# kfirc1503/generative-audio

Hardware: AMD Instinct MI355X
Metric: spectrogram-frames/sec, NPPC K=5 FullSubNet+ train step (higher is better)
Workload: dtype bf16

## Files before the change

generative-audio_amd/csrc/spec.hip:

```cpp
#include "common.h"
#include "nppc_hip.h"

namespace {

struct MapSet { const float* x[6]; };

template <bool RAGGED>
__global__ __launch_bounds__(256) void rowsum_kernel(MapSet ms, double* __restrict__ sums, const int* __restrict__ frames, long R,
                                                     int C, int T) {
  const long r = (long)blockIdx.x * 4 + (threadIdx.x >> 6);
  if (r >= R) return;
  const int lane = threadIdx.x & 63;
  const int Tb = RAGGED ? clampi(frames[r / C], 1, T) : T;
  const float* x = ms.x[blockIdx.y];
  sums += (size_t)blockIdx.y * R;
  const float* p = x + (size_t)r * T;
  double s = 0.0;
  for (int t = lane; t < Tb; t += 64) s += (double)p[t];
  s = wave_sum(s);
  if (lane == 0) sums[r] = s;
}

struct TsseW {
  const float* cw[3];
  const float* cb[3];
  int ks[3];
  const float* fcw;
  const float* fcb;
  const float* w1;
  const float* b1;
  const float* w2;
  const float* b2;
};

constexpr int TSSE_MAXC = 1024;
__device__ __forceinline__ TsseW tsse_branch(TsseW w, long off) {
  for (int i = 0; i < 3; ++i) { w.cw[i] += off; if (w.cb[i]) w.cb[i] += off; }
  w.fcw += off; if (w.fcb) w.fcb += off;
  w.w1 += off; if (w.b1) w.b1 += off;
  w.w2 += off; if (w.b2) w.b2 += off;
  return w;
}

template <bool RAGGED>
__global__ __launch_bounds__(1024) void tsse_fwd_kernel(MapSet ms, const double* __restrict__ rowsum,
                                                       TsseW w, long sW, int nm, float* __restrict__ scale, float* __restrict__ ns_out,
                                                       float* __restrict__ pre_out, float* __restrict__ sq_out,
                                                       float* __restrict__ h1_out, float* __restrict__ sg_out,
                                                       const int* __restrict__ frames, int C, int C2, int T, int la) {
  __shared__ double red[16];
  __shared__ float sq[TSSE_MAXC];
  __shared__ float h1[TSSE_MAXC / 2];
  __shared__ float ns_s;
  const int b = blockIdx.x, tid = threadIdx.x;
  {
    const int j = blockIdx.y, z = j % 3, m = j / 3, B = gridDim.x;
    const size_t slot = (size_t)z * nm + m;
    w = tsse_branch(w, (long)z * sW);
    rowsum += (size_t)j * B * C;
    scale += slot * B * C;
    if (ns_out) ns_out += slot * B;
    if (pre_out) pre_out += slot * B * C * 3;
    if (sq_out) sq_out += slot * B * C;
    if (h1_out) h1_out += slot * B * C2;
    if (sg_out) sg_out += slot * B * C;
  }
  const float* __restrict__ x = ms.x[blockIdx.y];
  const int Tn = RAGGED ? clampi(frames[b], 1, T) : T;
  const int Tp = Tn + la;
  double part = 0.0;
  for (int c = tid; c < C; c += blockDim.x) part += rowsum[(size_t)b * C + c];
  part = wave_sum(part);
  if ((tid & 63) == 0) red[tid >> 6] = part;
  __syncthreads();
  if (tid == 0) {
    double tot_all = 0.0;
    for (int wv = 0; wv < (int)(blockDim.x >> 6); ++wv) tot_all += red[wv];
    const float mu = (float)(tot_all / ((double)C * Tp));
    ns_s = 1.0f / (mu + 1e-5f);
    if (ns_out) ns_out[b] = ns_s;
  }
  __syncthreads();
  const float ns = ns_s;
  for (int c = tid; c < C; c += blockDim.x) {
    const float* xr = x + ((size_t)b * C + c) * T;
    const double tot = rowsum[(size_t)b * C + c];
    float acc = w.fcb[0];
    for (int i = 0; i < 3; ++i) {
      const int ks = w.ks[i];
      const int Lout = Tp - ks + 1;
      double conv = 0.0;
      for (int k = 0; k < ks; ++k) {
        double pre = 0.0, suf = 0.0;
        for (int t = 0; t < k; ++t) pre += (t < Tn) ? (double)xr[t] : 0.0;
        for (int m = 0; m < ks - 1 - k; ++m) {
          const int t = Tp - 1 - m;
          suf += (t < Tn && t >= 0) ? (double)xr[t] : 0.0;
        }
        conv += (double)w.cw[i][c * ks + k] * (tot - pre - suf);
      }
      const float pv = w.cb[i][c] + ns * (float)(conv / Lout);
      if (pre_out) pre_out[((size_t)b * C + c) * 3 + i] = pv;
      acc += w.fcw[i] * fmaxf(pv, 0.f);
    }
    sq[c] = acc;
    if (sq_out) sq_out[(size_t)b * C + c] = acc;
  }
  __syncthreads();
  for (int j = tid; j < C2; j += blockDim.x) {
    float a = w.b1[j];
    const float* wr = w.w1 + (size_t)j * C;
    for (int c = 0; c < C; ++c) a += wr[c] * sq[c];
    a = fmaxf(a, 0.f);
    h1[j] = a;
    if (h1_out) h1_out[(size_t)b * C2 + j] = a;
  }
  __syncthreads();
  for (int c = tid; c < C; c += blockDim.x) {
    float a = w.b2[c];
    const float* wr = w.w2 + (size_t)c * C2;
    for (int j = 0; j < C2; ++j) a += wr[j] * h1[j];
    const float sg = 1.0f / (1.0f + expf(-a));
    if (sg_out) sg_out[(size_t)b * C + c] = sg;
    scale[(size_t)b * C + c] = ns * sg;
  }
}

template <typename T, bool RAGGED>
__global__ __launch_bounds__(256) void scale_transpose_kernel(MapSet ms, const float* __restrict__ scale,
                                                              T* __restrict__ y, const int* __restrict__ frames, int B, int nm,
                                                              long sY, int C, int Tn, int Tp, int ld, int coff) {
  __shared__ float tile[32][33];
  const int j = blockIdx.z / B, b = blockIdx.z % B, c0 = blockIdx.y * 32, t0 = blockIdx.x * 32;
  const float* __restrict__ x = ms.x[j];
  {
    const int z = j % 3, m = j / 3;
    if (scale) scale += ((size_t)z * nm + m) * B * C;
    y += (size_t)z * sY;
    coff += m * C;
  }
  const int Tb = RAGGED ? clampi(frames[b], 1, Tn) : Tn;
  const int Tw = RAGGED ? Tp : Tn;
  const int tx = threadIdx.x & 31, ty = threadIdx.x >> 5;
  for (int i = ty; i < 32; i += 8) {
    const int c = c0 + i, t = t0 + tx;
    float v = 0.f;
    if (c < C && t < Tb) {
      v = x[((size_t)b * C + c) * Tn + t];
      if (scale) v *= scale[(size_t)b * C + c];
    }
    tile[i][tx] = v;
  }
  __syncthreads();
  for (int i = ty; i < 32; i += 8) {
    const int t = t0 + i, c = c0 + tx;
    if (t < Tw && c < C) y[((size_t)b * Tp + t) * ld + coff + c] = from_f32<T>(tile[tx][i]);
  }
}

__host__ __device__ __forceinline__ long tsse_ws_stride(int B, int C, int KS) { return (long)B * (5L * C + C / 2 + (long)C * KS + 4); }

template <typename T>
__global__ __launch_bounds__(256) void tsse_bwd_ds_kernel(const T* __restrict__ dX0, MapSet ms,
                                                          const float* __restrict__ ns, float* __restrict__ dsg, int B, int nm,
                                                          long sY, long sWs, int C, int Tn, int Tp, int ld, int coff) {
  __shared__ float xt[64][65];
  __shared__ float part[4][64];
  const int j = blockIdx.z / B, b = blockIdx.z % B, c0 = blockIdx.x * 64, tid = threadIdx.x;
  const float* __restrict__ x = ms.x[j];
  {
    const int z = j % 3, m = j / 3;
    dX0 += (size_t)z * sY;
    coff += m * C;
    ns += ((size_t)z * nm + m) * B;
    dsg += (size_t)j * sWs;
  }
  const int cl = tid & 63, tl = tid >> 6;
  float s = 0.f;
  for (int t0 = 0; t0 < Tn; t0 += 64) {
    __syncthreads();
    for (int e = tid; e < 64 * 64; e += 256) {
      const int cc = e / 64, tt = e % 64;
      xt[cc][tt] = (c0 + cc < C && t0 + tt < Tn) ? x[((size_t)b * C + c0 + cc) * Tn + t0 + tt] : 0.f;
    }
    __syncthreads();
    if (c0 + cl < C) {
      const T* dp = dX0 + (size_t)b * Tp * ld + coff + c0 + cl;
#pragma unroll 4
      for (int k = 0; k < 16; ++k) {
        const int tt = tl + 4 * k;
        if (t0 + tt < Tn) s += to_f32<T>(dp[(size_t)(t0 + tt) * ld]) * xt[cl][tt];
      }
    }
  }
  part[tl][cl] = s;
  __syncthreads();
  if (tid < 64 && c0 + tid < C)
    dsg[(size_t)b * C + c0 + tid] = ns[b] * (((part[0][tid] + part[1][tid]) + part[2][tid]) + part[3][tid]);
}

struct TsseG {
  float* cw[3];
  float* cb[3];
  float* fcw; float* fcb; float* w1; float* b1; float* w2; float* b2;
};

__device__ __forceinline__ TsseG tsse_branch_g(TsseG g, long off) {
  for (int i = 0; i < 3; ++i) { g.cw[i] += off; g.cb[i] += off; }
  g.fcw += off; g.fcb += off; g.w1 += off; g.b1 += off; g.w2 += off; g.b2 += off;
  return g;
}

__global__ __launch_bounds__(1024) void tsse_bwd_mlp_kernel(MapSet ms, const double* __restrict__ rowsum,
                                                           TsseW w, long sW, int nm, const float* __restrict__ ns_in,
                                                           const float* __restrict__ pre, const float* __restrict__ sq,
                                                           const float* __restrict__ h1, const float* __restrict__ sg,
                                                           float* __restrict__ ws, long sWs, int C, int C2, int T, int la) {
  __shared__ float da2[TSSE_MAXC];
  __shared__ float da1[TSSE_MAXC / 2];
  __shared__ float wsum[4][16];
  const int b = blockIdx.x, tid = threadIdx.x;
  const int B = gridDim.x;
  const int KS = w.ks[0] + w.ks[1] + w.ks[2];
  const float* __restrict__ x = ms.x[blockIdx.y];
  float* __restrict__ wj = ws + (size_t)blockIdx.y * sWs;
  const float* __restrict__ dsg = wj;
  float* __restrict__ da2_ws = wj + (size_t)B * C;
  float* __restrict__ da1_ws = da2_ws + (size_t)B * C;
  float* __restrict__ pcb = da1_ws + (size_t)B * C2 + (size_t)b * 3 * C;
  float* __restrict__ pcw = da1_ws + (size_t)B * C2 + (size_t)B * 3 * C + (size_t)b * C * KS;
  float* __restrict__ pf = da1_ws + (size_t)B * C2 + (size_t)B * 3 * C + (size_t)B * C * KS + (size_t)b * 4;
  {
    const int j = blockIdx.y, z = j % 3, m = j / 3;
    const size_t slot = (size_t)z * nm + m;
    w = tsse_branch(w, (long)z * sW);
    rowsum += (size_t)j * B * C;
    ns_in += slot * B;
    pre += slot * B * C * 3;
    sq += slot * B * C;
    h1 += slot * B * C2;
    sg += slot * B * C;
  }
  const int Tp = T + la;
  const float ns = ns_in[b];
  for (int c = tid; c < C; c += blockDim.x) {
    const float s = sg[(size_t)b * C + c];
    const float d = dsg[(size_t)b * C + c] * s * (1.f - s);
    da2[c] = d;
    da2_ws[(size_t)b * C + c] = d;
  }
  __syncthreads();
  for (int j = tid; j < C2; j += blockDim.x) {
    float a = 0.f;
    for (int c = 0; c < C; ++c) a += w.w2[(size_t)c * C2 + j] * da2[c];
    a = h1[(size_t)b * C2 + j] > 0.f ? a : 0.f;
    da1[j] = a;
    da1_ws[(size_t)b * C2 + j] = a;
  }
  __syncthreads();
  float fsum[3] = {0.f, 0.f, 0.f}, bsum = 0.f;
  for (int c = tid; c < C; c += blockDim.x) {
    float a = 0.f;
    for (int j = 0; j < C2; ++j) a += w.w1[(size_t)j * C + c] * da1[j];
    bsum += a;
    const float* xr = x + ((size_t)b * C + c) * T;
    const double tot = rowsum[(size_t)b * C + c];
    int koff = 0;
    for (int i = 0; i < 3; ++i) {
      const float pv = pre[((size_t)b * C + c) * 3 + i];
      fsum[i] += a * fmaxf(pv, 0.f);
      const float dp = pv > 0.f ? a * w.fcw[i] : 0.f;
      pcb[i * C + c] = dp;
      const int ks = w.ks[i];
      const int Lout = Tp - ks + 1;
      for (int k = 0; k < ks; ++k) {
        float v = 0.f;
        if (dp != 0.f) {
          double prf = 0.0, suf = 0.0;
          for (int t = 0; t < k; ++t) prf += (t < T) ? (double)xr[t] : 0.0;
          for (int m = 0; m < ks - 1 - k; ++m) {
            const int t = Tp - 1 - m;
            suf += (t < T && t >= 0) ? (double)xr[t] : 0.0;
          }
          v = dp * ns * (float)((tot - prf - suf) / Lout);
        }
        pcw[(size_t)C * koff + c * ks + k] = v;
      }
      koff += ks;
    }
  }
  for (int i = 0; i < 4; ++i) {
    const float v = wave_sum(i < 3 ? fsum[i] : bsum);
    if ((tid & 63) == 0) wsum[i][tid >> 6] = v;
  }
  __syncthreads();
  if (tid < 4) {
    float v = 0.f;
    for (int wv = 0; wv < (int)(blockDim.x >> 6); ++wv) v += wsum[tid][wv];
    pf[tid] = v;
  }
}

__global__ __launch_bounds__(256) void tsse_bwd_outer_kernel(const float* __restrict__ ws, long sWs,
                                                             const float* __restrict__ h1, const float* __restrict__ sq, TsseG g,
                                                             long sW, int nm, int B, int C, int C2, int ks0, int ks1, int ks2,
                                                             int map0 ) {
  const int z = blockIdx.y;
  g = tsse_branch_g(g, (long)z * sW);
  const int KS = ks0 + ks1 + ks2;
  const int n2 = C * C2;
  const long nW = (long)C * KS;
  const long e = (long)blockIdx.x * 256 + threadIdx.x;
  const long total = 2L * n2 + C + C2 + 3L * C + nW + 4;
  if (e >= total) return;
  float* dst;
  {
    long k = e;
    if (k < n2) dst = g.w2 + k;
    else if ((k -= n2) < n2) dst = g.w1 + k;
    else if ((k -= n2) < C) dst = g.b2 + k;
    else if ((k -= C) < C2) dst = g.b1 + k;
    else if ((k -= C2) < 3L * C) dst = g.cb[k / C] + k % C;
    else if ((k -= 3L * C) < nW) {
      if (k < (long)C * ks0) dst = g.cw[0] + k;
      else if (k < (long)C * (ks0 + ks1)) dst = g.cw[1] + (k - (long)C * ks0);
      else dst = g.cw[2] + (k - (long)C * (ks0 + ks1));
    } else { k -= nW; dst = k < 3 ? g.fcw + k : g.fcb; }
  }
  float acc = *dst;
  for (int m = 0; m < nm; ++m) {
    const int j = map0 >= 0 ? map0 : m * 3 + z;
    const size_t slot = map0 >= 0 ? 0 : (size_t)z * nm + m;
    const float* __restrict__ da2 = ws + (size_t)j * sWs + (size_t)B * C;
    const float* __restrict__ da1 = da2 + (size_t)B * C;
    const float* __restrict__ pcb = da1 + (size_t)B * C2;
    const float* __restrict__ pcw = pcb + (size_t)B * 3 * C;
    const float* __restrict__ pf = pcw + (size_t)B * nW;
    const float* __restrict__ h1m = h1 + slot * B * C2;
    const float* __restrict__ sqm = sq + slot * B * C;
    float a = 0.f;
    long k = e;
    if (k < n2) {
      const int c = (int)(k / C2), jj = (int)(k % C2);
      for (int b = 0; b < B; ++b) a += da2[(size_t)b * C + c] * h1m[(size_t)b * C2 + jj];
    } else if ((k -= n2) < n2) {
      const int jj = (int)(k / C), c = (int)(k % C);
      for (int b = 0; b < B; ++b) a += da1[(size_t)b * C2 + jj] * sqm[(size_t)b * C + c];
    } else if ((k -= n2) < C) {
      for (int b = 0; b < B; ++b) a += da2[(size_t)b * C + k];
    } else if ((k -= C) < C2) {
      for (int b = 0; b < B; ++b) a += da1[(size_t)b * C2 + k];
    } else if ((k -= C2) < 3L * C) {
      for (int b = 0; b < B; ++b) a += pcb[(size_t)b * 3 * C + k];
    } else if ((k -= 3L * C) < nW) {
      for (int b = 0; b < B; ++b) a += pcw[(size_t)b * nW + k];
    } else {
      k -= nW;
      for (int b = 0; b < B; ++b) a += pf[(size_t)b * 4 + k];
    }
    acc += a;
  }
  *dst = acc;
}

template <bool RAGGED>
int tsse_fwd_maps(int prec, const float* const* maps, int nmaps, double* rowsum, const TsseW& w, long sW, float* scale, float* ns,
                  float* pre, float* sq, float* h1, float* sg, void* X0, long sY, const int* frames, int B, int C, int T,
                  int look_ahead, int Tp, int ld, void* stream) {
  if (!maps || !rowsum || !scale || !X0 || B <= 0 || C <= 0 || C > TSSE_MAXC || (nmaps != 3 && nmaps != 6)) return NPPC_EBADARG;
  if (w.ks[0] > T || w.ks[1] > T || w.ks[2] > T) return NPPC_EUNSUPPORTED;
  const int nm = nmaps / 3;
  if (nm * C > ld || T > Tp) return NPPC_EBADARG;
  hipStream_t s = (hipStream_t)stream;
  MapSet ms{};
  for (int j = 0; j < nmaps; ++j) { if (!maps[j]) return NPPC_EBADARG; ms.x[j] = maps[j]; }
  hipLaunchKernelGGL(rowsum_kernel<RAGGED>, dim3(ceil_div((long)B * C, 4), nmaps), dim3(256), 0, s, ms, rowsum, frames,
                     (long)B * C, C, T);
  const int nt = round_up(C, 64) > 1024 ? 1024 : round_up(C, 64);
  hipLaunchKernelGGL(tsse_fwd_kernel<RAGGED>, dim3(B, nmaps), dim3(nt), 0, s, ms, rowsum, w, sW, nm, scale, ns, pre, sq, h1, sg,
                     frames, C, C / 2, T, look_ahead);
  dim3 grid(ceil_div(RAGGED ? Tp : T, 32), ceil_div(C, 32), B * nmaps);
  if (prec == NPPC_PREC_BF16)
    hipLaunchKernelGGL((scale_transpose_kernel<bf16_t, RAGGED>), grid, dim3(256), 0, s, ms, scale, (bf16_t*)X0, frames, B, nm, sY, C,
                       T, Tp, ld, 0);
  else if (prec == NPPC_PREC_F32)
    hipLaunchKernelGGL((scale_transpose_kernel<float, RAGGED>), grid, dim3(256), 0, s, ms, scale, (float*)X0, frames, B, nm, sY, C, T,
                       Tp, ld, 0);
  else
    return NPPC_EBADARG;
  NPPC_CHECK_LAUNCH();
  return NPPC_OK;
}

}

extern "C" {

int nppc_tsse_bwd_maps(int prec, const void* dX0, long sY, const float* const* maps, int nmaps, const double* rowsum,
                       const float* cw0, const float* cw1, const float* cw2, int ks0, int ks1, int ks2, const float* fcw,
                       const float* w1, const float* w2, long sW, const float* ns, const float* pre, const float* sq,
                       const float* h1, const float* sg, float* ws, float* g_cw0, float* g_cb0, float* g_cw1, float* g_cb1,
                       float* g_cw2, float* g_cb2, float* g_fcw, float* g_fcb, float* g_w1, float* g_b1, float* g_w2, float* g_b2,
                       int B, int C, int T, int look_ahead, int Tp, int ld, void* stream) {
  if (!dX0 || !maps || !rowsum || !ws || B <= 0 || C > TSSE_MAXC || (nmaps != 3 && nmaps != 6)) return NPPC_EBADARG;
  hipStream_t s = (hipStream_t)stream;
  MapSet ms{};
  for (int j = 0; j < nmaps; ++j) { if (!maps[j]) return NPPC_EBADARG; ms.x[j] = maps[j]; }
  const int nm = nmaps / 3, C2 = C / 2, KS = ks0 + ks1 + ks2;
  const long sWs = tsse_ws_stride(B, C, KS);
  dim3 g1(ceil_div(C, 64), 1, B * nmaps);
  if (prec == NPPC_PREC_BF16)
    hipLaunchKernelGGL(tsse_bwd_ds_kernel<bf16_t>, g1, dim3(256), 0, s, (const bf16_t*)dX0, ms, ns, ws, B, nm, sY, sWs, C, T, Tp, ld, 0);
  else
    hipLaunchKernelGGL(tsse_bwd_ds_kernel<float>, g1, dim3(256), 0, s, (const float*)dX0, ms, ns, ws, B, nm, sY, sWs, C, T, Tp, ld, 0);
  TsseW w{{cw0, cw1, cw2}, {nullptr, nullptr, nullptr}, {ks0, ks1, ks2}, fcw, nullptr, w1, nullptr, w2, nullptr};
  TsseG g{{g_cw0, g_cw1, g_cw2}, {g_cb0, g_cb1, g_cb2}, g_fcw, g_fcb, g_w1, g_b1, g_w2, g_b2};
  const int nt = round_up(C, 64) > 1024 ? 1024 : round_up(C, 64);
  hipLaunchKernelGGL(tsse_bwd_mlp_kernel, dim3(B, nmaps), dim3(nt), 0, s, ms, rowsum, w, sW, nm, ns, pre, sq, h1, sg, ws, sWs, C,
                     C2, T, look_ahead);
  const long total = 2L * C * C2 + C + C2 + 3L * C + (long)C * KS + 4;
  hipLaunchKernelGGL(tsse_bwd_outer_kernel, dim3(ceil_div(total, 256), 3), dim3(256), 0, s, ws, sWs, h1, sq, g, sW, nm, B, C, C2,
                     ks0, ks1, ks2, -1);
  NPPC_CHECK_LAUNCH();
  return NPPC_OK;
}

int nppc_tsse_fwd_maps(int prec, const float* const* maps, int nmaps, double* rowsum, const float* cw0, const float* cb0,
                       const float* cw1, const float* cb1, const float* cw2, const float* cb2, int ks0, int ks1, int ks2,
                       const float* fcw, const float* fcb, const float* w1, const float* b1, const float* w2, const float* b2, long sW,
                       float* scale, float* ns, float* pre, float* sq, float* h1, float* sg, void* X0, long sY, int B, int C, int T,
                       int look_ahead, int Tp, int ld, void* stream) {
  const TsseW w{{cw0, cw1, cw2}, {cb0, cb1, cb2}, {ks0, ks1, ks2}, fcw, fcb, w1, b1, w2, b2};
  return tsse_fwd_maps<false>(prec, maps, nmaps, rowsum, w, sW, scale, ns, pre, sq, h1, sg, X0, sY, nullptr, B, C, T, look_ahead,
                              Tp, ld, stream);
}

int nppc_tsse_fwd_maps_ragged(int prec, const float* const* maps, int nmaps, double* rowsum, const float* cw0, const float* cb0,
                              const float* cw1, const float* cb1, const float* cw2, const float* cb2, int ks0, int ks1, int ks2,
                              const float* fcw, const float* fcb, const float* w1, const float* b1, const float* w2,
                              const float* b2, long sW, float* scale, void* X0, long sY, const int* frames, int B, int C, int T,
                              int look_ahead, int Tp, int ld, void* stream) {
  if (!frames || !cw0 || !cb0 || !cw1 || !cb1 || !cw2 || !cb2 || !fcw || !fcb || !w1 || !b1 || !w2 || !b2) return NPPC_EBADARG;
  const TsseW w{{cw0, cw1, cw2}, {cb0, cb1, cb2}, {ks0, ks1, ks2}, fcw, fcb, w1, b1, w2, b2};
  return tsse_fwd_maps<true>(prec, maps, nmaps, rowsum, w, sW, scale, nullptr, nullptr, nullptr, nullptr, nullptr, X0, sY, frames,
                             B, C, T, look_ahead, Tp, ld, stream);
}

int nppc_tsse_bwd(int prec, const void* dX0, const float* x, const double* rowsum, const float* cw0, const float* cw1,
                  const float* cw2, int ks0, int ks1, int ks2, const float* fcw, const float* w1, const float* w2,
                  const float* ns, const float* pre, const float* sq, const float* h1, const float* sg, float* dsg_ws,
                  float* g_cw0, float* g_cb0, float* g_cw1, float* g_cb1, float* g_cw2, float* g_cb2, float* g_fcw,
                  float* g_fcb, float* g_w1, float* g_b1, float* g_w2, float* g_b2, int B, int C, int T, int look_ahead, int Tp,
                  int ld, int coff, void* stream) {
  if (!dX0 || !x || !rowsum || !dsg_ws || B <= 0 || C > TSSE_MAXC) return NPPC_EBADARG;
  hipStream_t s = (hipStream_t)stream;
  dim3 g1(ceil_div(C, 64), 1, B);
  MapSet ms{};
  ms.x[0] = x;
  const int C2 = C / 2, KS = ks0 + ks1 + ks2;
  const long sWs1 = tsse_ws_stride(B, C, KS);
  if (prec == NPPC_PREC_BF16)
    hipLaunchKernelGGL(tsse_bwd_ds_kernel<bf16_t>, g1, dim3(256), 0, s, (const bf16_t*)dX0, ms, ns, dsg_ws, B, 1, 0L, sWs1, C, T, Tp, ld, coff);
  else
    hipLaunchKernelGGL(tsse_bwd_ds_kernel<float>, g1, dim3(256), 0, s, (const float*)dX0, ms, ns, dsg_ws, B, 1, 0L, sWs1, C, T, Tp, ld, coff);
  TsseW w{{cw0, cw1, cw2}, {nullptr, nullptr, nullptr}, {ks0, ks1, ks2}, fcw, nullptr, w1, nullptr, w2, nullptr};
  TsseG g{{g_cw0, g_cw1, g_cw2}, {g_cb0, g_cb1, g_cb2}, g_fcw, g_fcb, g_w1, g_b1, g_w2, g_b2};
  const int nt = round_up(C, 64) > 1024 ? 1024 : round_up(C, 64);
  hipLaunchKernelGGL(tsse_bwd_mlp_kernel, dim3(B, 1), dim3(nt), 0, s, ms, rowsum, w, 0L, 1, ns, pre, sq, h1, sg, dsg_ws, sWs1,
                     C, C2, T, look_ahead);
  const long total = 2L * C * C2 + C + C2 + 3L * C + (long)C * KS + 4;
  hipLaunchKernelGGL(tsse_bwd_outer_kernel, dim3(ceil_div(total, 256), 1), dim3(256), 0, s, dsg_ws, sWs1, h1, sq, g, 0L, 1, B, C, C2,
                     ks0, ks1, ks2, 0);
  NPPC_CHECK_LAUNCH();
  return NPPC_OK;
}

int nppc_tsse_bwd_ws_elems(int nmaps, int B, int C, int ks0, int ks1, int ks2, long* elems) {
  if (!elems || nmaps < 1 || B < 1 || C < 1) return NPPC_EBADARG;
  *elems = (long)nmaps * tsse_ws_stride(B, C, ks0 + ks1 + ks2);
  return NPPC_OK;
}

int nppc_rowsum(const float* x, double* sums, long R, int T, void* stream) {
  if (!x || !sums || R <= 0 || T <= 0) return NPPC_EBADARG;
  MapSet ms{};
  ms.x[0] = x;
  hipLaunchKernelGGL(rowsum_kernel<false>, dim3(ceil_div(R, 4), 1), dim3(256), 0, (hipStream_t)stream, ms, sums, nullptr, R, 0, T);
  NPPC_CHECK_LAUNCH();
  return NPPC_OK;
}

int nppc_tsse_fwd(const float* x, const double* rowsum, const float* cw0, const float* cb0, const float* cw1,
                  const float* cb1, const float* cw2, const float* cb2, int ks0, int ks1, int ks2, const float* fcw,
                  const float* fcb, const float* w1, const float* b1, const float* w2, const float* b2, float* scale,
                  float* ns, float* pre, float* sq, float* h1, float* sg, int B, int C, int T, int look_ahead,
                  void* stream) {
  if (!x || !rowsum || !scale || B <= 0 || C <= 0 || C > TSSE_MAXC) return NPPC_EBADARG;
  if (ks0 > T || ks1 > T || ks2 > T) return NPPC_EUNSUPPORTED;
  TsseW w{{cw0, cw1, cw2}, {cb0, cb1, cb2}, {ks0, ks1, ks2}, fcw, fcb, w1, b1, w2, b2};
  const int nt = round_up(C, 64) > 1024 ? 1024 : round_up(C, 64);
  MapSet ms{};
  ms.x[0] = x;
  hipLaunchKernelGGL(tsse_fwd_kernel<false>, dim3(B, 1), dim3(nt), 0, (hipStream_t)stream, ms, rowsum, w, 0L, 1, scale, ns, pre, sq, h1,
                     sg, nullptr, C, C / 2, T, look_ahead);
  NPPC_CHECK_LAUNCH();
  return NPPC_OK;
}

int nppc_scale_transpose(int prec, const float* x, const float* scale, void* y, int B, int C, int T, int Tp, int ld,
                         int coff, void* stream) {
  if (!x || !y || B <= 0 || coff + C > ld || T > Tp) return NPPC_EBADARG;
  dim3 grid(ceil_div(T, 32), ceil_div(C, 32), B);
  MapSet ms{};
  ms.x[0] = x;
  if (prec == NPPC_PREC_BF16)
    hipLaunchKernelGGL((scale_transpose_kernel<bf16_t, false>), grid, dim3(256), 0, (hipStream_t)stream, ms, scale, (bf16_t*)y,
                       nullptr, B, 1, 0L, C, T, Tp, ld, coff);
  else if (prec == NPPC_PREC_F32)
    hipLaunchKernelGGL((scale_transpose_kernel<float, false>), grid, dim3(256), 0, (hipStream_t)stream, ms, scale, (float*)y,
                       nullptr, B, 1, 0L, C, T, Tp, ld, coff);
  else
    return NPPC_EBADARG;
  NPPC_CHECK_LAUNCH();
  return NPPC_OK;
}

}
```

Before: 259,100.

## Fuse rowsum into TSSE forward, stage edges and MLP weights in LDS, retile backward ds

The forward TSSE kernel now computes the per-row sums itself, so the separate rowsum launch goes away. It caches the leading and trailing edge samples in dynamic LDS, which removes the repeated global reads in the O(ks^2) prefix/suffix loops. The two MLP matvecs now stream weights through LDS tiles with register prefetch instead of each thread reading uncoalesced rows. The backward ds kernel is rewritten around 8-column chunks with vectorised bf16 loads, a software-pipelined request/stage loop and a different block size. The costs are large dynamic LDS use, fixed 1024-thread blocks, and extra host-side LDS capacity checks that can reject configurations.

Result: no change. 259,400 (median of 3 runs) (+0.1%).

```diff
diff --git a/generative-audio_amd/csrc/spec.hip b/generative-audio_amd/csrc/spec.hip
--- a/generative-audio_amd/csrc/spec.hip
+++ b/generative-audio_amd/csrc/spec.hip
@@ -1,3 +1,5 @@
+#include <type_traits>
+
 #include "common.h"
 #include "nppc_hip.h"
 
@@ -5,18 +7,13 @@
 
 struct MapSet { const float* x[6]; };
 
-template <bool RAGGED>
-__global__ __launch_bounds__(256) void rowsum_kernel(MapSet ms, double* __restrict__ sums, const int* __restrict__ frames, long R,
-                                                     int C, int T) {
+__global__ __launch_bounds__(256) void rowsum_kernel(const float* __restrict__ x, double* __restrict__ sums, long R, int T) {
   const long r = (long)blockIdx.x * 4 + (threadIdx.x >> 6);
   if (r >= R) return;
   const int lane = threadIdx.x & 63;
-  const int Tb = RAGGED ? clampi(frames[r / C], 1, T) : T;
-  const float* x = ms.x[blockIdx.y];
-  sums += (size_t)blockIdx.y * R;
   const float* p = x + (size_t)r * T;
   double s = 0.0;
-  for (int t = lane; t < Tb; t += 64) s += (double)p[t];
+  for (int t = lane; t < T; t += 64) s += (double)p[t];
   s = wave_sum(s);
   if (lane == 0) sums[r] = s;
 }
@@ -34,6 +31,17 @@
 };
 
 constexpr int TSSE_MAXC = 1024;
+constexpr int TSSE_NT = 1024;
+constexpr int TSSE_WTILE = 9 * TSSE_NT;
+constexpr int TSSE_WREGS = TSSE_WTILE / TSSE_NT;
+constexpr int TSSE_KREG = 16;
+constexpr size_t TSSE_MAX_LDS = 160 * 1024 - 1024;
+
+__host__ __device__ __forceinline__ size_t tsse_fwd_lds_bytes(int C, int E) {
+  const size_t edges = 2 * (size_t)E * C;
+  return 8 * (size_t)C + 4 * ((size_t)C + C / 2 + (edges > (size_t)TSSE_WTILE ? edges : (size_t)TSSE_WTILE));
+}
+
 __device__ __forceinline__ TsseW tsse_branch(TsseW w, long off) {
   for (int i = 0; i < 3; ++i) { w.cw[i] += off; if (w.cb[i]) w.cb[i] += off; }
   w.fcw += off; if (w.fcb) w.fcb += off;
@@ -42,22 +50,120 @@
   return w;
 }
 
+__device__ __forceinline__ void tsse_load_edges(const float* __restrict__ xr, float* ef, float* el, int c, int C, int E, int Tn,
+                                                int Tp) {
+  for (int k = 0; k < E; ++k) {
+    const int t = Tp - 1 - k;
+    ef[k * C + c] = k < Tn ? xr[k] : 0.f;
+    el[k * C + c] = (t < Tn && t >= 0) ? xr[t] : 0.f;
+  }
+}
+
+__device__ __forceinline__ double tsse_window_sum(const float* ef, const float* el, int c, int C, int k, int ks, double tot,
+                                                  double& prf) {
+  if (k > 0) prf += (double)ef[(k - 1) * C + c];
+  double suf = 0.0;
+#pragma unroll 4
+  for (int m = 0; m < ks - 1 - k; ++m) suf += (double)el[m * C + c];
+  return tot - prf - suf;
+}
+
+__device__ __forceinline__ float tsse_matvec(const float* __restrict__ W, int n_out, int n_in, const float* v, float a,
+                                             float* tile) {
+  const int tid = threadIdx.x;
+  if (n_out <= 0 || n_in <= 0) return a;
+  int lg = 6;
+  while (lg > 3 && n_out * ((1 << lg) + 1) > TSSE_WTILE) --lg;
+  const int KT = 1 << lg, ldt = KT + 1;
+  float r[TSSE_WREGS];
+  auto request = [&](int k0) {
+#pragma unroll
+    for (int u = 0; u < TSSE_WREGS; ++u) {
+      const int e = tid + u * TSSE_NT, o = e >> lg, k = k0 + (e & (KT - 1));
+      r[u] = (o < n_out && k < n_in) ? W[(size_t)o * n_in + k] : 0.f;
+    }
+  };
+  request(0);
+  for (int k0 = 0; k0 < n_in; k0 += KT) {
+    const int kn = n_in - k0 < KT ? n_in - k0 : KT;
+    __syncthreads();
+#pragma unroll
+    for (int u = 0; u < TSSE_WREGS; ++u) {
+      const int e = tid + u * TSSE_NT, o = e >> lg;
+      if (o < n_out) tile[o * ldt + (e & (KT - 1))] = r[u];
+    }
+    __syncthreads();
+    if (k0 + KT < n_in) request(k0 + KT);
+    if (tid < n_out) {
+      const float* tr = tile + tid * ldt;
+      const float* vk = v + k0;
+#pragma unroll 16
+      for (int k = 0; k < kn; ++k) a = fmaf(tr[k], vk[k], a);
+    }
+  }
+  __syncthreads();
+  return a;
+}
+
+__device__ __forceinline__ float tsse_matvec_t(const float* __restrict__ W, int n_out, int n_in, const float* v, float a,
+                                               float* tile) {
+  const int tid = threadIdx.x;
+  if (n_out <= 0 || n_in <= 0) return a;
+  const int RT = TSSE_WTILE / n_out;
+  float r[TSSE_WREGS];
+  auto request = [&](int r0) {
+    const int n = (n_in - r0 < RT ? n_in - r0 : RT) * n_out;
+    const float* __restrict__ src = W + (size_t)r0 * n_out;
+#pragma unroll
+    for (int u = 0; u < TSSE_WREGS; ++u) {
+      const int e = tid + u * TSSE_NT;
+      r[u] = e < n ? src[e] : 0.f;
+    }
+  };
+  request(0);
+  for (int r0 = 0; r0 < n_in; r0 += RT) {
+    const int rn = n_in - r0 < RT ? n_in - r0 : RT;
+    __syncthreads();
+#pragma unroll
+    for (int u = 0; u < TSSE_WREGS; ++u) {
+      const int e = tid + u * TSSE_NT;
+      if (e < rn * n_out) tile[e] = r[u];
+    }
+    __syncthreads();
+    if (r0 + RT < n_in) request(r0 + RT);
+    if (tid < n_out) {
+      const float* tc = tile + tid;
+      const float* vr = v + r0;
+#pragma unroll 16
+      for (int i = 0; i < rn; ++i) a = fmaf(tc[i * n_out], vr[i], a);
+    }
+  }
+  __syncthreads();
+  return a;
+}
+
 template <bool RAGGED>
-__global__ __launch_bounds__(1024) void tsse_fwd_kernel(MapSet ms, const double* __restrict__ rowsum,
-                                                       TsseW w, long sW, int nm, float* __restrict__ scale, float* __restrict__ ns_out,
-                                                       float* __restrict__ pre_out, float* __restrict__ sq_out,
-                                                       float* __restrict__ h1_out, float* __restrict__ sg_out,
-                                                       const int* __restrict__ frames, int C, int C2, int T, int la) {
-  __shared__ double red[16];
-  __shared__ float sq[TSSE_MAXC];
-  __shared__ float h1[TSSE_MAXC / 2];
+__global__ __launch_bounds__(TSSE_NT) void tsse_fwd_kernel(MapSet ms, double* __restrict__ rowsum, const double* __restrict__ rowsum_in,
+                                                          TsseW w, long sW, int nm, float* __restrict__ scale, float* __restrict__ ns_out,
+                                                          float* __restrict__ pre_out, float* __restrict__ sq_out,
+                                                          float* __restrict__ h1_out, float* __restrict__ sg_out,
+                                                          const int* __restrict__ frames, int C, int C2, int T, int la, int E) {
+  extern __shared__ double tsse_lds[];
+  __shared__ double red[TSSE_NT / 64];
   __shared__ float ns_s;
-  const int b = blockIdx.x, tid = threadIdx.x;
+  double* rs = tsse_lds;
+  float* sq = reinterpret_cast<float*>(rs + C);
+  float* h1 = sq + C;
+  float* ef = h1 + C2;
+  float* el = ef + (size_t)E * C;
+  float* tile = ef;
+  const int b = blockIdx.x, tid = threadIdx.x, lane = tid & 63, wv = tid >> 6;
   {
     const int j = blockIdx.y, z = j % 3, m = j / 3, B = gridDim.x;
     const size_t slot = (size_t)z * nm + m;
     w = tsse_branch(w, (long)z * sW);
-    rowsum += (size_t)j * B * C;
+    if (rowsum) rowsum += (size_t)j * B * C;
+    if (rowsum_in) rowsum_in += (size_t)j * B * C;
     scale += slot * B * C;
     if (ns_out) ns_out += slot * B;
     if (pre_out) pre_out += slot * B * C * 3;
@@ -65,64 +171,111 @@
     if (h1_out) h1_out += slot * B * C2;
     if (sg_out) sg_out += slot * B * C;
   }
-  const float* __restrict__ x = ms.x[blockIdx.y];
   const int Tn = RAGGED ? clampi(frames[b], 1, T) : T;
   const int Tp = Tn + la;
-  double part = 0.0;
-  for (int c = tid; c < C; c += blockDim.x) part += rowsum[(size_t)b * C + c];
-  part = wave_sum(part);
-  if ((tid & 63) == 0) red[tid >> 6] = part;
+  const float* __restrict__ xb = ms.x[blockIdx.y] + (size_t)b * C * T;
+  if (rowsum_in) {
+    if (tid < C) {
+      rs[tid] = rowsum_in[(size_t)b * C + tid];
+      tsse_load_edges(xb + (size_t)tid * T, ef, el, tid, C, E, Tn, Tp);
+    }
+  } else {
+    for (int i = tid; i < 2 * E * C; i += TSSE_NT) ef[i] = 0.f;
+    __syncthreads();
+    for (int r0 = wv * 8; r0 < C; r0 += (TSSE_NT / 64) * 8) {
+      double s[8];
+#pragma unroll
+      for (int q = 0; q < 8; ++q) s[q] = 0.0;
+      for (int t = lane; t < Tn; t += 128) {
+        float v[2][8];
+#pragma unroll
+        for (int h = 0; h < 2; ++h)
+#pragma unroll
+          for (int q = 0; q < 8; ++q) v[h][q] = (r0 + q < C && t + 64 * h < Tn) ? xb[(size_t)(r0 + q) * T + t + 64 * h] : 0.f;
+#pragma unroll
+        for (int h = 0; h < 2; ++h) {
+          const int th = t + 64 * h, mlast = Tp - 1 - th;
+          if (th < Tn) {
+#pragma unroll
+            for (int q = 0; q < 8; ++q) {
+              s[q] += (double)v[h][q];
+              if (r0 + q < C) {
+                if (th < E) ef[th * C + r0 + q] = v[h][q];
+                if (mlast < E) el[mlast * C + r0 + q] = v[h][q];
+              }
+            }
+          }
+        }
+      }
+#pragma unroll
+      for (int q = 0; q < 8; ++q) {
+        if (r0 + q < C) {
+          const double tot = wave_sum(s[q]);
+          if (lane == 0) { rs[r0 + q] = tot; rowsum[(size_t)b * C + r0 + q] = tot; }
+        }
+      }
+    }
+  }
+  __syncthreads();
+  {
+    double part = tid < C ? rs[tid] : 0.0;
+    part = wave_sum(part);
+    if (lane == 0) red[wv] = part;
+  }
   __syncthreads();
   if (tid == 0) {
     double tot_all = 0.0;
-    for (int wv = 0; wv < (int)(blockDim.x >> 6); ++wv) tot_all += red[wv];
+    for (int i = 0; i < (C + 63) / 64; ++i) tot_all += red[i];
     const float mu = (float)(tot_all / ((double)C * Tp));
     ns_s = 1.0f / (mu + 1e-5f);
     if (ns_out) ns_out[b] = ns_s;
   }
   __syncthreads();
   const float ns = ns_s;
-  for (int c = tid; c < C; c += blockDim.x) {
-    const float* xr = x + ((size_t)b * C + c) * T;
-    const double tot = rowsum[(size_t)b * C + c];
+  if (tid < C) {
+    const int c = tid;
+    float wk[3][TSSE_KREG], cb[3], fw[3];
+#pragma unroll
+    for (int i = 0; i < 3; ++i) {
+#pragma unroll
+      for (int k = 0; k < TSSE_KREG; ++k) wk[i][k] = k < w.ks[i] ? w.cw[i][c * w.ks[i] + k] : 0.f;
+      cb[i] = w.cb[i][c];
+      fw[i] = w.fcw[i];
+    }
+    const double tot = rs[c];
     float acc = w.fcb[0];
+#pragma unroll
     for (int i = 0; i < 3; ++i) {
       const int ks = w.ks[i];
       const int Lout = Tp - ks + 1;
-      double conv = 0.0;
-      for (int k = 0; k < ks; ++k) {
-        double pre = 0.0, suf = 0.0;
-        for (int t = 0; t < k; ++t) pre += (t < Tn) ? (double)xr[t] : 0.0;
-        for (int m = 0; m < ks - 1 - k; ++m) {
-          const int t = Tp - 1 - m;
-          suf += (t < Tn && t >= 0) ? (double)xr[t] : 0.0;
-        }
-        conv += (double)w.cw[i][c * ks + k] * (tot - pre - suf);
-      }
-      const float pv = w.cb[i][c] + ns * (float)(conv / Lout);
+      double conv = 0.0, prf = 0.0;
+#pragma unroll
+      for (int k = 0; k < TSSE_KREG; ++k)
+        if (k < ks) conv += (double)wk[i][k] * tsse_window_sum(ef, el, c, C, k, ks, tot, prf);
+      for (int k = TSSE_KREG; k < ks; ++k)
+        conv += (double)w.cw[i][c * ks + k] * tsse_window_sum(ef, el, c, C, k, ks, tot, prf);
+      const float pv = cb[i] + ns * (float)(conv / Lout);
       if (pre_out) pre_out[((size_t)b * C + c) * 3 + i] = pv;
-      acc += w.fcw[i] * fmaxf(pv, 0.f);
+      acc += fw[i] * fmaxf(pv, 0.f);
     }
     sq[c] = acc;
     if (sq_out) sq_out[(size_t)b * C + c] = acc;
   }
-  __syncthreads();
-  for (int j = tid; j < C2; j += blockDim.x) {
-    float a = w.b1[j];
-    const float* wr = w.w1 + (size_t)j * C;
-    for (int c = 0; c < C; ++c) a += wr[c] * sq[c];
-    a = fmaxf(a, 0.f);
-    h1[j] = a;
-    if (h1_out) h1_out[(size_t)b * C2 + j] = a;
-  }
-  __syncthreads();
-  for (int c = tid; c < C; c += blockDim.x) {
-    float a = w.b2[c];
-    const float* wr = w.w2 + (size_t)c * C2;
-    for (int j = 0; j < C2; ++j) a += wr[j] * h1[j];
-    const float sg = 1.0f / (1.0f + expf(-a));
-    if (sg_out) sg_out[(size_t)b * C + c] = sg;
-    scale[(size_t)b * C + c] = ns * sg;
+  {
+    float a = tsse_matvec(w.w1, C2, C, sq, tid < C2 ? w.b1[tid] : 0.f, tile);
+    if (tid < C2) {
+      a = fmaxf(a, 0.f);
+      h1[tid] = a;
+      if (h1_out) h1_out[(size_t)b * C2 + tid] = a;
+    }
+  }
+  {
+    const float a = tsse_matvec(w.w2, C, C2, h1, tid < C ? w.b2[tid] : 0.f, tile);
+    if (tid < C) {
+      const float sg = 1.0f / (1.0f + expf(-a));
+      if (sg_out) sg_out[(size_t)b * C + tid] = sg;
+      scale[(size_t)b * C + tid] = ns * sg;
+    }
   }
 }
 
@@ -160,43 +313,137 @@
 
 __host__ __device__ __forceinline__ long tsse_ws_stride(int B, int C, int KS) { return (long)B * (5L * C + C / 2 + (long)C * KS + 4); }
 
-template <typename T>
-__global__ __launch_bounds__(256) void tsse_bwd_ds_kernel(const T* __restrict__ dX0, MapSet ms,
-                                                          const float* __restrict__ ns, float* __restrict__ dsg, int B, int nm,
-                                                          long sY, long sWs, int C, int Tn, int Tp, int ld, int coff) {
-  __shared__ float xt[64][65];
-  __shared__ float part[4][64];
-  const int j = blockIdx.z / B, b = blockIdx.z % B, c0 = blockIdx.x * 64, tid = threadIdx.x;
-  const float* __restrict__ x = ms.x[j];
-  {
-    const int z = j % 3, m = j / 3;
-    dX0 += (size_t)z * sY;
-    coff += m * C;
-    ns += ((size_t)z * nm + m) * B;
-    dsg += (size_t)j * sWs;
-  }
-  const int cl = tid & 63, tl = tid >> 6;
+constexpr int DS_CH = 9, DS_W = 8 * DS_CH, DS_NT = 320, DS_NW = DS_NT / 64;
+constexpr int DS_XR = (DS_W + DS_NW - 1) / DS_NW;
+
+template <typename T, bool VEC>
+__global__ __launch_bounds__(DS_NT) void tsse_bwd_ds_kernel(const T* __restrict__ dX0, MapSet ms,
+                                                            const float* __restrict__ ns, float* __restrict__ dsg, int B, int nm,
+                                                            long sY, long sWs, int C, int Tn, int Tp, int ld, int coff,
+                                                            int chunk0, int nch) {
+  constexpr int NV = 16 / (int)sizeof(T);
+  constexpr int LPC = 8 / NV;
+  constexpr int ND = VEC ? (64 * DS_CH * LPC + DS_NT - 1) / DS_NT : (64 * DS_W + DS_NT - 1) / DS_NT;
+  __shared__ float xt[DS_W][65];
+  __shared__ __attribute__((aligned(16))) float dt[64][DS_W];
+  __shared__ float part[4][DS_W];
+  const int z = blockIdx.z / B, b = blockIdx.z % B, tid = threadIdx.x, lane = tid & 63, wv = tid >> 6;
+  const int G = gridDim.x, g = blockIdx.x;
+  const int ch_lo = (int)((long)g * nch / G), ch_hi = (int)((long)(g + 1) * nch / G);
+  const int col0 = 8 * (chunk0 + ch_lo), wd = 8 * (ch_hi - ch_lo), W = nm * C;
+  if (wd <= 0) return;
+  dX0 += (size_t)z * sY + (size_t)b * Tp * ld;
+
+  const float* xp[DS_XR];
+#pragma unroll
+  for (int u = 0; u < DS_XR; ++u) {
+    const int cc = wv + DS_NW * u, rel = col0 + cc - coff;
+    xp[u] = nullptr;
+    if (cc < wd && rel >= 0 && rel < W) {
+      const int m = rel >= C, c = rel - m * C;
+      xp[u] = ms.x[m * 3 + z] + ((size_t)b * C + c) * Tn + lane;
+    }
+  }
+  int dtt[ND], dcc[ND];
+#pragma unroll
+  for (int u = 0; u < ND; ++u) {
+    const int e = tid + DS_NT * u;
+    if constexpr (VEC) {
+      const int per = (wd / 8) * LPC;
+      dtt[u] = e / per;
+      dcc[u] = (e - dtt[u] * per) * NV;
+    } else {
+      dtt[u] = e / wd;
+      dcc[u] = e - dtt[u] * wd;
+      const int rel = col0 + dcc[u] - coff;
+      if (rel < 0 || rel >= W) dtt[u] = 64;
+    }
+    if (dtt[u] > 64) dtt[u] = 64;
+  }
+  float xr[DS_XR];
+  typename std::conditional<VEC, uint4, float>::type dr[ND];
+  auto request = [&](int t0) {
+#pragma unroll
+    for (int u = 0; u < DS_XR; ++u) xr[u] = (xp[u] && t0 + lane < Tn) ? xp[u][t0] : 0.f;
+#pragma unroll
+    for (int u = 0; u < ND; ++u) {
+      const bool on = dtt[u] < 64 && t0 + dtt[u] < Tn;
+      const T* src = dX0 + (size_t)(t0 + dtt[u]) * ld + col0 + dcc[u];
+      if constexpr (VEC) dr[u] = on ? *reinterpret_cast<const uint4*>(src) : uint4{0u, 0u, 0u, 0u};
+      else dr[u] = on ? to_f32<T>(*src) : 0.f;
+    }
+  };
+  auto stage = [&]() {
+#pragma unroll
+    for (int u = 0; u < DS_XR; ++u) {
+      const int cc = wv + DS_NW * u;
+      if (cc < wd) xt[cc][lane] = xr[u];
+    }
+#pragma unroll
+    for (int u = 0; u < ND; ++u) {
+      if (dtt[u] >= 64) continue;
+      float* o = &dt[dtt[u]][dcc[u]];
+      if constexpr (VEC) {
+        const unsigned wds[4] = {dr[u].x, dr[u].y, dr[u].z, dr[u].w};
+        if constexpr (sizeof(T) == 2) {
+#pragma unroll
+          for (int i = 0; i < 4; ++i) {
+            o[2 * i] = __uint_as_float(wds[i] << 16);
+            o[2 * i + 1] = __uint_as_float(wds[i] & 0xffff0000u);
+          }
+        } else {
+#pragma unroll
+          for (int i = 0; i < 4; ++i) o[i] = __uint_as_float(wds[i]);
+        }
+      } else {
+        *o = dr[u];
+      }
+    }
+  };
+
+  const int cl = tid % DS_W, tl = tid / DS_W;
+  const int rel = col0 + cl - coff;
+  const bool mine = tl < 4 && cl < wd && rel >= 0 && rel < W;
   float s = 0.f;
+  request(0);
   for (int t0 = 0; t0 < Tn; t0 += 64) {
     __syncthreads();
-    for (int e = tid; e < 64 * 64; e += 256) {
-      const int cc = e / 64, tt = e % 64;
-      xt[cc][tt] = (c0 + cc < C && t0 + tt < Tn) ? x[((size_t)b * C + c0 + cc) * Tn + t0 + tt] : 0.f;
-    }
+    stage();
     __syncthreads();
-    if (c0 + cl < C) {
-      const T* dp = dX0 + (size_t)b * Tp * ld + coff + c0 + cl;
-#pragma unroll 4
+    if (t0 + 64 < Tn) request(t0 + 64);
+    if (mine) {
+#pragma unroll
       for (int k = 0; k < 16; ++k) {
         const int tt = tl + 4 * k;
-        if (t0 + tt < Tn) s += to_f32<T>(dp[(size_t)(t0 + tt) * ld]) * xt[cl][tt];
+        if (t0 + tt < Tn) s += dt[tt][cl] * xt[cl][tt];
       }
     }
   }
-  part[tl][cl] = s;
+  if (tl < 4) part[tl][cl] = s;
   __syncthreads();
-  if (tid < 64 && c0 + tid < C)
-    dsg[(size_t)b * C + c0 + tid] = ns[b] * (((part[0][tid] + part[1][tid]) + part[2][tid]) + part[3][tid]);
+  if (tid < wd) {
+    const int r = col0 + tid - coff;
+    if (r >= 0 && r < W) {
+      const int m = r >= C, c = r - m * C;
+      dsg[(size_t)(m * 3 + z) * sWs + (size_t)b * C + c] =
+          ns[((size_t)z * nm + m) * B + b] * (((part[0][tid] + part[1][tid]) + part[2][tid]) + part[3][tid]);
+    }
+  }
+}
+
+template <typename T>
+void launch_tsse_bwd_ds(const T* dX0, const MapSet& ms, const float* ns, float* dsg, int B, int nm, int nz, long sY, long sWs,
+                        int C, int Tn, int Tp, int ld, int coff, hipStream_t s) {
+  const int chunk0 = coff / 8, nch = (coff + nm * C - 1) / 8 - chunk0 + 1;
+  dim3 grid(ceil_div(nch, DS_CH), 1, B * nz);
+  const long per16 = 16 / (long)sizeof(T);
+  const bool vec = ((uintptr_t)dX0 % 16 == 0) && ld % 8 == 0 && sY % per16 == 0;
+  if (vec)
+    hipLaunchKernelGGL((tsse_bwd_ds_kernel<T, true>), grid, dim3(DS_NT), 0, s, dX0, ms, ns, dsg, B, nm, sY, sWs, C, Tn, Tp, ld,
+                       coff, chunk0, nch);
+  else
+    hipLaunchKernelGGL((tsse_bwd_ds_kernel<T, false>), grid, dim3(DS_NT), 0, s, dX0, ms, ns, dsg, B, nm, sY, sWs, C, Tn, Tp, ld,
+                       coff, chunk0, nch);
 }
 
 struct TsseG {
@@ -211,14 +458,20 @@
   return g;
 }
 
-__global__ __launch_bounds__(1024) void tsse_bwd_mlp_kernel(MapSet ms, const double* __restrict__ rowsum,
+__global__ __launch_bounds__(TSSE_NT) void tsse_bwd_mlp_kernel(MapSet ms, const double* __restrict__ rowsum,
                                                            TsseW w, long sW, int nm, const float* __restrict__ ns_in,
                                                            const float* __restrict__ pre, const float* __restrict__ sq,
                                                            const float* __restrict__ h1, const float* __restrict__ sg,
-                                                           float* __restrict__ ws, long sWs, int C, int C2, int T, int la) {
+                                                           float* __restrict__ ws, long sWs, int C, int C2, int T, int la, int E) {
+  extern __shared__ double tsse_edges[];
   __shared__ float da2[TSSE_MAXC];
   __shared__ float da1[TSSE_MAXC / 2];
   __shared__ float wsum[4][16];
+  double* totl = tsse_edges;
+  float* tile = reinterpret_cast<float*>(totl + C);
+  float* ef = tile + TSSE_WTILE;
+  float* el = ef + (size_t)E * C;
+  float* dpl = el + (size_t)E * C;
   const int b = blockIdx.x, tid = threadIdx.x;
   const int B = gridDim.x;
   const int KS = w.ks[0] + w.ks[1] + w.ks[2];
@@ -243,50 +496,37 @@
   }
   const int Tp = T + la;
   const float ns = ns_in[b];
-  for (int c = tid; c < C; c += blockDim.x) {
+  float pv[3] = {0.f, 0.f, 0.f};
+  if (tid < C) {
+    const int c = tid;
     const float s = sg[(size_t)b * C + c];
     const float d = dsg[(size_t)b * C + c] * s * (1.f - s);
+    for (int i = 0; i < 3; ++i) pv[i] = pre[((size_t)b * C + c) * 3 + i];
+    totl[c] = rowsum[(size_t)b * C + c];
     da2[c] = d;
     da2_ws[(size_t)b * C + c] = d;
-  }
-  __syncthreads();
-  for (int j = tid; j < C2; j += blockDim.x) {
-    float a = 0.f;
-    for (int c = 0; c < C; ++c) a += w.w2[(size_t)c * C2 + j] * da2[c];
-    a = h1[(size_t)b * C2 + j] > 0.f ? a : 0.f;
-    da1[j] = a;
-    da1_ws[(size_t)b * C2 + j] = a;
-  }
-  __syncthreads();
+    tsse_load_edges(x + ((size_t)b * C + c) * T, ef, el, c, C, E, T, Tp);
+  }
+  {
+    float a = tsse_matvec_t(w.w2, C2, C, da2, 0.f, tile);
+    if (tid < C2) {
+      a = h1[(size_t)b * C2 + tid] > 0.f ? a : 0.f;
+      da1[tid] = a;
+      da1_ws[(size_t)b * C2 + tid] = a;
+    }
+  }
   float fsum[3] = {0.f, 0.f, 0.f}, bsum = 0.f;
-  for (int c = tid; c < C; c += blockDim.x) {
-    float a = 0.f;
-    for (int j = 0; j < C2; ++j) a += w.w1[(size_t)j * C + c] * da1[j];
-    bsum += a;
-    const float* xr = x + ((size_t)b * C + c) * T;
-    const double tot = rowsum[(size_t)b * C + c];
-    int koff = 0;
-    for (int i = 0; i < 3; ++i) {
-      const float pv = pre[((size_t)b * C + c) * 3 + i];
-      fsum[i] += a * fmaxf(pv, 0.f);
-      const float dp = pv > 0.f ? a * w.fcw[i] : 0.f;
-      pcb[i * C + c] = dp;
-      const int ks = w.ks[i];
-      const int Lout = Tp - ks + 1;
-      for (int k = 0; k < ks; ++k) {
-        float v = 0.f;
-        if (dp != 0.f) {
-          double prf = 0.0, suf = 0.0;
-          for (int t = 0; t < k; ++t) prf += (t < T) ? (double)xr[t] : 0.0;
-          for (int m = 0; m < ks - 1 - k; ++m) {
-            const int t = Tp - 1 - m;
-            suf += (t < T && t >= 0) ? (double)xr[t] : 0.0;
-          }
-          v = dp * ns * (float)((tot - prf - suf) / Lout);
-        }
-        pcw[(size_t)C * koff + c * ks + k] = v;
+  {
+    const float a = tsse_matvec_t(w.w1, C, C2, da1, 0.f, tile);
+    if (tid < C) {
+      const int c = tid;
+      bsum += a;
+      for (int i = 0; i < 3; ++i) {
+        fsum[i] += a * fmaxf(pv[i], 0.f);
+        const float dp = pv[i] > 0.f ? a * w.fcw[i] : 0.f;
+        pcb[i * C + c] = dp;
+        dpl[i * C + c] = dp;
       }
-      koff += ks;
     }
   }
   for (int i = 0; i < 4; ++i) {
@@ -296,9 +536,59 @@
   __syncthreads();
   if (tid < 4) {
     float v = 0.f;
-    for (int wv = 0; wv < (int)(blockDim.x >> 6); ++wv) v += wsum[tid][wv];
+    for (int wv = 0; wv < (C + 63) / 64; ++wv) v += wsum[tid][wv];
     pf[tid] = v;
   }
+  int koff = 0;
+  for (int i = 0; i < 3; ++i) {
+    const int ks = w.ks[i];
+    const int Lout = Tp - ks + 1;
+    for (int e = tid; e < C * ks; e += TSSE_NT) {
+      const int c = e / ks, k = e - c * ks;
+      const float dp = dpl[i * C + c];
+      float v = 0.f;
+      if (dp != 0.f) {
+        double prf = 0.0;
+#pragma unroll 4
+        for (int t = 0; t < k; ++t) prf += (double)ef[t * C + c];
+        double suf = 0.0;
+#pragma unroll 4
+        for (int m = 0; m < ks - 1 - k; ++m) suf += (double)el[m * C + c];
+        v = dp * ns * (float)((totl[c] - prf - suf) / Lout);
+      }
+      pcw[(size_t)C * koff + e] = v;
+    }
+    koff += ks;
+  }
+}
+
+constexpr int TSSE_OB = 16;
+__device__ __forceinline__ float tsse_dot_samples(const float* __restrict__ p, size_t sp, const float* __restrict__ q, size_t sq,
+                                                  int B) {
+  float a = 0.f;
+  int b = 0;
+  for (; b + TSSE_OB <= B; b += TSSE_OB) {
+    float u[TSSE_OB], v[TSSE_OB];
+#pragma unroll
+    for (int i = 0; i < TSSE_OB; ++i) { u[i] = p[(size_t)(b + i) * sp]; v[i] = q[(size_t)(b + i) * sq]; }
+#pragma unroll
+    for (int i = 0; i < TSSE_OB; ++i) a = fmaf(u[i], v[i], a);
+  }
+  for (; b < B; ++b) a = fmaf(p[(size_t)b * sp], q[(size_t)b * sq], a);
+  return a;
+}
+__device__ __forceinline__ float tsse_sum_samples(const float* __restrict__ p, size_t sp, int B) {
+  float a = 0.f;
+  int b = 0;
+  for (; b + TSSE_OB <= B; b += TSSE_OB) {
+    float u[TSSE_OB];
+#pragma unroll
+    for (int i = 0; i < TSSE_OB; ++i) u[i] = p[(size_t)(b + i) * sp];
+#pragma unroll
+    for (int i = 0; i < TSSE_OB; ++i) a += u[i];
+  }
+  for (; b < B; ++b) a += p[(size_t)b * sp];
+  return a;
 }
 
 __global__ __launch_bounds__(256) void tsse_bwd_outer_kernel(const float* __restrict__ ws, long sWs,
@@ -338,29 +628,67 @@
     const float* __restrict__ pf = pcw + (size_t)B * nW;
     const float* __restrict__ h1m = h1 + slot * B * C2;
     const float* __restrict__ sqm = sq + slot * B * C;
-    float a = 0.f;
+    float a;
     long k = e;
     if (k < n2) {
       const int c = (int)(k / C2), jj = (int)(k % C2);
-      for (int b = 0; b < B; ++b) a += da2[(size_t)b * C + c] * h1m[(size_t)b * C2 + jj];
+      a = tsse_dot_samples(da2 + c, C, h1m + jj, C2, B);
     } else if ((k -= n2) < n2) {
       const int jj = (int)(k / C), c = (int)(k % C);
-      for (int b = 0; b < B; ++b) a += da1[(size_t)b * C2 + jj] * sqm[(size_t)b * C + c];
+      a = tsse_dot_samples(da1 + jj, C2, sqm + c, C, B);
     } else if ((k -= n2) < C) {
-      for (int b = 0; b < B; ++b) a += da2[(size_t)b * C + k];
+      a = tsse_sum_samples(da2 + k, C, B);
     } else if ((k -= C) < C2) {
-      for (int b = 0; b < B; ++b) a += da1[(size_t)b * C2 + k];
+      a = tsse_sum_samples(da1 + k, C2, B);
     } else if ((k -= C2) < 3L * C) {
-      for (int b = 0; b < B; ++b) a += pcb[(size_t)b * 3 * C + k];
+      a = tsse_sum_samples(pcb + k, 3 * (size_t)C, B);
     } else if ((k -= 3L * C) < nW) {
-      for (int b = 0; b < B; ++b) a += pcw[(size_t)b * nW + k];
+      a = tsse_sum_samples(pcw + k, nW, B);
     } else {
       k -= nW;
-      for (int b = 0; b < B; ++b) a += pf[(size_t)b * 4 + k];
+      a = tsse_sum_samples(pf + k, 4, B);
     }
     acc += a;
   }
   *dst = acc;
+}
+
+inline int tsse_lds_ok(const void* kernel, size_t bytes) {
+  if (bytes > TSSE_MAX_LDS) return NPPC_EUNSUPPORTED;
+  if (bytes > 64 * 1024 &&
+      hipFuncSetAttribute(kernel, hipFuncAttributeMaxDynamicSharedMemorySize, (int)bytes) != hipSuccess)
+    return NPPC_ELAUNCH;
+  return NPPC_OK;
+}
+
+inline int tsse_edge(int ks0, int ks1, int ks2) {
+  const int k = ks0 > ks1 ? (ks0 > ks2 ? ks0 : ks2) : (ks1 > ks2 ? ks1 : ks2);
+  return k > 1 ? k - 1 : 0;
+}
+
+template <bool RAGGED>
+int launch_tsse_fwd(const MapSet& ms, int nmaps, double* rowsum, const double* rowsum_in, const TsseW& w, long sW, int nm,
+                    float* scale, float* ns, float* pre, float* sq, float* h1, float* sg, const int* frames, int B, int C, int T,
+                    int look_ahead, hipStream_t s) {
+  const int E = tsse_edge(w.ks[0], w.ks[1], w.ks[2]);
+  const size_t lds = tsse_fwd_lds_bytes(C, E);
+  const int rc = tsse_lds_ok(reinterpret_cast<const void*>(&tsse_fwd_kernel<RAGGED>), lds);
+  if (rc != NPPC_OK) return rc;
+  hipLaunchKernelGGL(tsse_fwd_kernel<RAGGED>, dim3(B, nmaps), dim3(TSSE_NT), lds, s, ms, rowsum, rowsum_in, w, sW, nm, scale, ns,
+                     pre, sq, h1, sg, frames, C, C / 2, T, look_ahead, E);
+  return NPPC_OK;
+}
+
+int launch_tsse_bwd_mlp(const MapSet& ms, int nmaps, const double* rowsum, const TsseW& w, long sW, int nm, const float* ns,
+                        const float* pre, const float* sq, const float* h1, const float* sg, float* ws, long sWs, int B, int C,
+                        int T, int look_ahead, hipStream_t s) {
+  const int E = tsse_edge(w.ks[0], w.ks[1], w.ks[2]);
+  const size_t lds = 8 * (size_t)C + 4 * ((size_t)TSSE_WTILE + 2 * (size_t)E * C + 3 * (size_t)C);
+  const int rc = tsse_lds_ok(reinterpret_cast<const void*>(&tsse_bwd_mlp_kernel), lds + 8 * 1024);
+  if (rc != NPPC_OK) return rc;
+  hipLaunchKernelGGL(tsse_bwd_mlp_kernel, dim3(B, nmaps), dim3(TSSE_NT), lds, s, ms, rowsum, w, sW, nm, ns, pre, sq, h1, sg, ws, sWs, C,
+                     C / 2, T, look_ahead, E);
+  return NPPC_OK;
 }
 
 template <bool RAGGED>
@@ -371,23 +699,20 @@
   if (w.ks[0] > T || w.ks[1] > T || w.ks[2] > T) return NPPC_EUNSUPPORTED;
   const int nm = nmaps / 3;
   if (nm * C > ld || T > Tp) return NPPC_EBADARG;
+  if (prec != NPPC_PREC_BF16 && prec != NPPC_PREC_F32) return NPPC_EBADARG;
   hipStream_t s = (hipStream_t)stream;
   MapSet ms{};
   for (int j = 0; j < nmaps; ++j) { if (!maps[j]) return NPPC_EBADARG; ms.x[j] = maps[j]; }
-  hipLaunchKernelGGL(rowsum_kernel<RAGGED>, dim3(ceil_div((long)B * C, 4), nmaps), dim3(256), 0, s, ms, rowsum, frames,
-                     (long)B * C, C, T);
-  const int nt = round_up(C, 64) > 1024 ? 1024 : round_up(C, 64);
-  hipLaunchKernelGGL(tsse_fwd_kernel<RAGGED>, dim3(B, nmaps), dim3(nt), 0, s, ms, rowsum, w, sW, nm, scale, ns, pre, sq, h1, sg,
-                     frames, C, C / 2, T, look_ahead);
+  const int rc = launch_tsse_fwd<RAGGED>(ms, nmaps, rowsum, nullptr, w, sW, nm, scale, ns, pre, sq, h1, sg, frames, B, C, T,
+                                         look_ahead, s);
+  if (rc != NPPC_OK) return rc;
   dim3 grid(ceil_div(RAGGED ? Tp : T, 32), ceil_div(C, 32), B * nmaps);
   if (prec == NPPC_PREC_BF16)
     hipLaunchKernelGGL((scale_transpose_kernel<bf16_t, RAGGED>), grid, dim3(256), 0, s, ms, scale, (bf16_t*)X0, frames, B, nm, sY, C,
                        T, Tp, ld, 0);
-  else if (prec == NPPC_PREC_F32)
+  else
     hipLaunchKernelGGL((scale_transpose_kernel<float, RAGGED>), grid, dim3(256), 0, s, ms, scale, (float*)X0, frames, B, nm, sY, C, T,
                        Tp, ld, 0);
-  else
-    return NPPC_EBADARG;
   NPPC_CHECK_LAUNCH();
   return NPPC_OK;
 }
@@ -402,22 +727,21 @@
                        const float* h1, const float* sg, float* ws, float* g_cw0, float* g_cb0, float* g_cw1, float* g_cb1,
                        float* g_cw2, float* g_cb2, float* g_fcw, float* g_fcb, float* g_w1, float* g_b1, float* g_w2, float* g_b2,
                        int B, int C, int T, int look_ahead, int Tp, int ld, void* stream) {
-  if (!dX0 || !maps || !rowsum || !ws || B <= 0 || C > TSSE_MAXC || (nmaps != 3 && nmaps != 6)) return NPPC_EBADARG;
+  if (!dX0 || !maps || !rowsum || !ws || B <= 0 || C <= 0 || C > TSSE_MAXC || (nmaps != 3 && nmaps != 6)) return NPPC_EBADARG;
+  if (nmaps / 3 * C > ld || T > Tp) return NPPC_EBADARG;
   hipStream_t s = (hipStream_t)stream;
   MapSet ms{};
   for (int j = 0; j < nmaps; ++j) { if (!maps[j]) return NPPC_EBADARG; ms.x[j] = maps[j]; }
   const int nm = nmaps / 3, C2 = C / 2, KS = ks0 + ks1 + ks2;
   const long sWs = tsse_ws_stride(B, C, KS);
-  dim3 g1(ceil_div(C, 64), 1, B * nmaps);
   if (prec == NPPC_PREC_BF16)
-    hipLaunchKernelGGL(tsse_bwd_ds_kernel<bf16_t>, g1, dim3(256), 0, s, (const bf16_t*)dX0, ms, ns, ws, B, nm, sY, sWs, C, T, Tp, ld, 0);
+    launch_tsse_bwd_ds((const bf16_t*)dX0, ms, ns, ws, B, nm, 3, sY, sWs, C, T, Tp, ld, 0, s);
   else
-    hipLaunchKernelGGL(tsse_bwd_ds_kernel<float>, g1, dim3(256), 0, s, (const float*)dX0, ms, ns, ws, B, nm, sY, sWs, C, T, Tp, ld, 0);
+    launch_tsse_bwd_ds((const float*)dX0, ms, ns, ws, B, nm, 3, sY, sWs, C, T, Tp, ld, 0, s);
   TsseW w{{cw0, cw1, cw2}, {nullptr, nullptr, nullptr}, {ks0, ks1, ks2}, fcw, nullptr, w1, nullptr, w2, nullptr};
   TsseG g{{g_cw0, g_cw1, g_cw2}, {g_cb0, g_cb1, g_cb2}, g_fcw, g_fcb, g_w1, g_b1, g_w2, g_b2};
-  const int nt = round_up(C, 64) > 1024 ? 1024 : round_up(C, 64);
-  hipLaunchKernelGGL(tsse_bwd_mlp_kernel, dim3(B, nmaps), dim3(nt), 0, s, ms, rowsum, w, sW, nm, ns, pre, sq, h1, sg, ws, sWs, C,
-                     C2, T, look_ahead);
+  const int rc = launch_tsse_bwd_mlp(ms, nmaps, rowsum, w, sW, nm, ns, pre, sq, h1, sg, ws, sWs, B, C, T, look_ahead, s);
+  if (rc != NPPC_OK) return rc;
   const long total = 2L * C * C2 + C + C2 + 3L * C + (long)C * KS + 4;
   hipLaunchKernelGGL(tsse_bwd_outer_kernel, dim3(ceil_div(total, 256), 3), dim3(256), 0, s, ws, sWs, h1, sq, g, sW, nm, B, C, C2,
                      ks0, ks1, ks2, -1);
@@ -452,22 +776,21 @@
                   float* g_cw0, float* g_cb0, float* g_cw1, float* g_cb1, float* g_cw2, float* g_cb2, float* g_fcw,
                   float* g_fcb, float* g_w1, float* g_b1, float* g_w2, float* g_b2, int B, int C, int T, int look_ahead, int Tp,
                   int ld, int coff, void* stream) {
-  if (!dX0 || !x || !rowsum || !dsg_ws || B <= 0 || C > TSSE_MAXC) return NPPC_EBADARG;
+  if (!dX0 || !x || !rowsum || !dsg_ws || B <= 0 || C <= 0 || C > TSSE_MAXC || coff < 0 || coff + C > ld || T > Tp)
+    return NPPC_EBADARG;
   hipStream_t s = (hipStream_t)stream;
-  dim3 g1(ceil_div(C, 64), 1, B);
   MapSet ms{};
   ms.x[0] = x;
   const int C2 = C / 2, KS = ks0 + ks1 + ks2;
   const long sWs1 = tsse_ws_stride(B, C, KS);
   if (prec == NPPC_PREC_BF16)
-    hipLaunchKernelGGL(tsse_bwd_ds_kernel<bf16_t>, g1, dim3(256), 0, s, (const bf16_t*)dX0, ms, ns, dsg_ws, B, 1, 0L, sWs1, C, T, Tp, ld, coff);
+    launch_tsse_bwd_ds((const bf16_t*)dX0, ms, ns, dsg_ws, B, 1, 1, 0L, sWs1, C, T, Tp, ld, coff, s);
   else
-    hipLaunchKernelGGL(tsse_bwd_ds_kernel<float>, g1, dim3(256), 0, s, (const float*)dX0, ms, ns, dsg_ws, B, 1, 0L, sWs1, C, T, Tp, ld, coff);
+    launch_tsse_bwd_ds((const float*)dX0, ms, ns, dsg_ws, B, 1, 1, 0L, sWs1, C, T, Tp, ld, coff, s);
   TsseW w{{cw0, cw1, cw2}, {nullptr, nullptr, nullptr}, {ks0, ks1, ks2}, fcw, nullptr, w1, nullptr, w2, nullptr};
   TsseG g{{g_cw0, g_cw1, g_cw2}, {g_cb0, g_cb1, g_cb2}, g_fcw, g_fcb, g_w1, g_b1, g_w2, g_b2};
-  const int nt = round_up(C, 64) > 1024 ? 1024 : round_up(C, 64);
-  hipLaunchKernelGGL(tsse_bwd_mlp_kernel, dim3(B, 1), dim3(nt), 0, s, ms, rowsum, w, 0L, 1, ns, pre, sq, h1, sg, dsg_ws, sWs1,
-                     C, C2, T, look_ahead);
+  const int rc = launch_tsse_bwd_mlp(ms, 1, rowsum, w, 0L, 1, ns, pre, sq, h1, sg, dsg_ws, sWs1, B, C, T, look_ahead, s);
+  if (rc != NPPC_OK) return rc;
   const long total = 2L * C * C2 + C + C2 + 3L * C + (long)C * KS + 4;
   hipLaunchKernelGGL(tsse_bwd_outer_kernel, dim3(ceil_div(total, 256), 1), dim3(256), 0, s, dsg_ws, sWs1, h1, sq, g, 0L, 1, B, C, C2,
                      ks0, ks1, ks2, 0);
@@ -483,9 +806,7 @@
 
 int nppc_rowsum(const float* x, double* sums, long R, int T, void* stream) {
   if (!x || !sums || R <= 0 || T <= 0) return NPPC_EBADARG;
-  MapSet ms{};
-  ms.x[0] = x;
-  hipLaunchKernelGGL(rowsum_kernel<false>, dim3(ceil_div(R, 4), 1), dim3(256), 0, (hipStream_t)stream, ms, sums, nullptr, R, 0, T);
+  hipLaunchKernelGGL(rowsum_kernel, dim3(ceil_div(R, 4)), dim3(256), 0, (hipStream_t)stream, x, sums, R, T);
   NPPC_CHECK_LAUNCH();
   return NPPC_OK;
 }
@@ -498,11 +819,11 @@
   if (!x || !rowsum || !scale || B <= 0 || C <= 0 || C > TSSE_MAXC) return NPPC_EBADARG;
   if (ks0 > T || ks1 > T || ks2 > T) return NPPC_EUNSUPPORTED;
   TsseW w{{cw0, cw1, cw2}, {cb0, cb1, cb2}, {ks0, ks1, ks2}, fcw, fcb, w1, b1, w2, b2};
-  const int nt = round_up(C, 64) > 1024 ? 1024 : round_up(C, 64);
   MapSet ms{};
   ms.x[0] = x;
-  hipLaunchKernelGGL(tsse_fwd_kernel<false>, dim3(B, 1), dim3(nt), 0, (hipStream_t)stream, ms, rowsum, w, 0L, 1, scale, ns, pre, sq, h1,
-                     sg, nullptr, C, C / 2, T, look_ahead);
+  const int rc = launch_tsse_fwd<false>(ms, 1, nullptr, rowsum, w, 0L, 1, scale, ns, pre, sq, h1, sg, nullptr, B, C, T, look_ahead,
+                                        (hipStream_t)stream);
+  if (rc != NPPC_OK) return rc;
   NPPC_CHECK_LAUNCH();
   return NPPC_OK;
 }
```
